# awkrail/svpc

Hardware: AMD Instinct MI355X
Metric: train steps/sec (vivt, batch=16, clip_seq=12) (higher is better)
Workload: dtype bf16x3; 1 GPU; MODEL_TYPE=vivt train step: N=16 videos/GPU x S=12 clips x Lv=100 frames x F=3072, Lt=22, D=768, H=12, L=6 (enc+step-enc+dec), V=951, A=384, E=10; dropout .1/.1/.4; fwd+bwd+allreduce+clip+BertAdam; mode=bf16x3, global_batch=16, parallelism=dp1, launch=hipGraph replay, gpus_requested=1

## Files before the change

include/svpc_hip.h:

```cpp
#ifndef SVPC_HIP_H
#define SVPC_HIP_H
#include <stddef.h>
#ifdef __cplusplus
extern "C" {
#endif

typedef struct ihipStream_t* svpc_stream_t;
typedef unsigned long long svpc_u64;

#define SVPC_ACT_NONE 0
#define SVPC_ACT_RELU 1
#define SVPC_ACT_GELU 2
#define SVPC_ACT_SIGMOID 3

const char* svpc_last_error(void);
int svpc_abi_version(void);

int svpc_ln_fwd(const float* x, const int* src_rows, const float* res, const float* gamma, const float* beta, float* y,
                float* mean, float* rstd, int R, int D, float eps, float p_pre, unsigned site_pre, float p_post,
                unsigned site_post, const svpc_u64* seed, const float* add1, int mod1, const float* add2, const int* idx2,
                svpc_stream_t stream);
int svpc_ln_fwd_t(const void* x, int x_dt, const int* src_rows, const void* res, const float* gamma, const float* beta, void* y,
                  int y_dt, float* mean, float* rstd, int R, int D, float eps, float p_pre, unsigned site_pre, float p_post,
                  unsigned site_post, const svpc_u64* seed, const float* add1, int mod1, const float* add2, const int* idx2,
// ... 64 lines not shown
int svpc_gemm_p8t(const void* A, int lda, const void* B, int ldb, void* C, int ldc, const void* G, int gact, const void* R, int M, int N, int K,
                  svpc_stream_t stream);
int svpc_gemm_l32_supported(int a_kc, int b_kc, int lda, int ldb, int M, int N, int K);
int svpc_gemm_l32_preferred(int a_kc, int b_kc, int lda, int ldb, int M, int N, int K);
int svpc_gemm_l32(const float* A, int lda, int a_kc, const float* B, int ldb, int b_kc, float* C, int ldc, float* Z, int M, int N, int K,
                  const float* bias, int act, float p_drop, unsigned site, const svpc_u64* seed, int accumulate, float* workspace,
                  size_t workspace_bytes, svpc_stream_t stream);
int svpc_gemm_l32_r(const float* A, int lda, int a_kc, const float* B, int ldb, int b_kc, float* C, int ldc, float* Z, const float* R, int M,
                    int N, int K, const float* bias, int act, float p_drop, unsigned site, const svpc_u64* seed, int accumulate,
                    float* workspace, size_t workspace_bytes, svpc_stream_t stream);
int svpc_gemm_l32_rg(const float* A, int lda, int a_kc, const float* B, int ldb, int b_kc, float* C, int ldc, const float* R, const float* G,
                     int gact, int M, int N, int K, int accumulate, float* workspace, size_t workspace_bytes, svpc_stream_t stream);
int svpc_gemm_l32_x3(const float* A, int lda, int a_kc, const float* B, int ldb, int b_kc, float* C, int ldc, float* Z, const float* R, int M,
                     int N, int K, const float* bias, int act, float p_drop, unsigned site, const svpc_u64* seed, int accumulate,
                     float* workspace, size_t workspace_bytes, svpc_stream_t stream);
typedef struct svpc_gemm_problem { const float* A; const float* B; float* C; int M, N, K, lda, ldb, ldc; } svpc_gemm_problem;
int svpc_gemm_group(const svpc_gemm_problem* problems, int n, int a_kc, int b_kc, int accumulate, svpc_stream_t stream);
int svpc_gemm_group_x3(const svpc_gemm_problem* problems, int n, int a_kc, int b_kc, int accumulate, svpc_stream_t stream);
typedef struct svpc_wgrad_problem {
    const float* dz; const float* x; float* dw; float* db;
    int n_out, n_in, rows, ld_dz, ld_x, ld_dw;
} svpc_wgrad_problem;
int svpc_gemm_group_wgrad_max(void);
int svpc_gemm_group_wgrad_bf16_p8_ok(const void* problems, int n);
int svpc_gemm_group_wgrad_bf16_p8(const void* problems, int n, float* workspace, size_t workspace_bytes, svpc_stream_t stream);
int svpc_gemm_group_wgrad_bf16(const svpc_wgrad_problem* problems, int n, svpc_stream_t stream);
int svpc_gemm_group_wgrad_bf16_ws(const svpc_wgrad_problem* problems, int n, float* workspace, size_t workspace_bytes,
                                  svpc_stream_t stream);
int svpc_gemm_group_wgrad(const svpc_wgrad_problem* problems, int n, svpc_stream_t stream);
int svpc_act_bwd(const float* dy, const float* aux, float* dz, size_t n, int act, float p, unsigned site, const svpc_u64* seed,
// ... 262 lines not shown
int svpc_scatter_add_rows_bf16(const float* rows, const int* idx, void* table, int ld_table, int R, int W, svpc_stream_t stream);
int svpc_pair_rows(float* a, const int* ia, float* b, const int* ib, float* out, float* out2, int R, int W, int mode, svpc_stream_t stream);
int svpc_add_cast_bf16(const void* a, const float* b, void* out, size_t n, svpc_stream_t stream);
int svpc_rows_expand(const float* src, const int* inv, float* out, int n_rows, int W, svpc_stream_t stream);
int svpc_add(const float* a, const float* b, float* c, size_t n, svpc_stream_t stream);
int svpc_sum_all(const float* x, size_t n, float* out, float scale, svpc_stream_t stream);
int svpc_fill_from(float* x, size_t n, const float* v, svpc_stream_t stream);
int svpc_dropout_mask(float* out, size_t n, float p, unsigned site, const svpc_u64* seed, svpc_stream_t stream);
int svpc_attn_dropout_mask(float* out, size_t n_rows, int max_k, float p, unsigned site, const svpc_u64* seed, svpc_stream_t stream);
int svpc_bump_seed(svpc_u64* seed, svpc_stream_t stream);

int svpc_opt_chunk(void);
int svpc_opt_meta_bytes(void);
int svpc_opt_step(const void* meta, const int* chunk_tid, const long long* chunk_start, const int* tensor_chunk_off, int n_tensors,
                  int n_chunks, float* partial, float* norms_sq, const float* hyper, svpc_stream_t stream);
int svpc_opt_zero_grad(const void* meta, const int* chunk_tid, const long long* chunk_start, int n_chunks, svpc_stream_t stream);

#ifdef __cplusplus
}
#endif
#endif
```

svpc_amd/csrc/gemm_l32.hip:

```cpp
#include "gemm_common.h"
#include <stdlib.h>

typedef __bf16 bf16x8 __attribute__((ext_vector_type(8)));
typedef const void __attribute__((address_space(1))) * l32_gptr;
typedef void __attribute__((address_space(3))) * l32_lptr;

constexpr int L32_BK = 32;
__device__ __attribute__((aligned(16))) const float l32_zeros[4] = {0.f, 0.f, 0.f, 0.f};

template <int N> __device__ __forceinline__ void l32_wait_vmcnt() { asm volatile("s_waitcnt vmcnt(%0)" ::"n"(N) : "memory"); }

template <int R, bool KC>
__device__ __forceinline__ const float* l32_src(const float* P, int ld, int m0, int rows, int k0, int j, int lane) {
    if (KC) {
        const int row = 8 * j + (lane >> 3), pos = lane & 7;
        const int c = pos ^ ((row >> 1) & 7);
        const int gr = min(m0 + row, rows - 1);
        return P + (size_t)gr * ld + k0 + 4 * c;
    } else {
        constexpr int CPR = R / 4;
        const int krow = j * (64 / CPR) + lane / CPR, c = lane % CPR;
        const int gm = min(m0 + 4 * c, rows - 4);
        return P + (size_t)(k0 + krow) * ld + gm;
    }
// ... 38 lines not shown
    } else {
        const float* p = reinterpret_cast<const float*>(img) + (16 * ks + 8 * (lane >> 5)) * R + row0 + (lane & 31);
#pragma unroll
        for (int j = 0; j < 8; ++j) f[j] = p[j * R];
    }
    l32_split8(f, hi, lo);
}
#define L32_MFMA3(ah, al, bh, bl, acc)                                           \
    do {                                                                         \
        acc = __builtin_amdgcn_mfma_f32_32x32x16_bf16(al, bh, acc, 0, 0, 0);     \
        acc = __builtin_amdgcn_mfma_f32_32x32x16_bf16(ah, bl, acc, 0, 0, 0);     \
        acc = __builtin_amdgcn_mfma_f32_32x32x16_bf16(ah, bh, acc, 0, 0, 0);     \
    } while (0)


template <int BM, int BN, bool A_KC, bool B_KC, int NS, bool X3 = false>
__global__ __launch_bounds__(256) void gemm_l32_kernel(const float* __restrict__ A, int lda, const float* __restrict__ B, int ldb,
                                                       float* __restrict__ C, int ldc, int M, int N, int K, Epi epi, int tiles_m,
                                                       int tiles_n, int splitk, int k_chunk, float* __restrict__ slabs, int remap) {
    extern __shared__ __attribute__((aligned(1024))) char l32_smem[];
    constexpr int A_BYTES = BM * L32_BK * 4, B_BYTES = BN * L32_BK * 4, STAGE = A_BYTES + B_BYTES;
    constexpr int A_PER_WAVE = BM / 32, B_PER_WAVE = BN / 32;
    constexpr int P = A_PER_WAVE + B_PER_WAVE;
    constexpr int TM = BM / 64, TN = BN / 64;
    const int wg = remap ? xcd_remap(blockIdx.x, tiles_m * tiles_n * splitk) : (int)blockIdx.x;
    const int ks_id = wg / (tiles_m * tiles_n);
    const int tile = wg - ks_id * (tiles_m * tiles_n);
    const int tm = tile / tiles_n, tn = tile - tm * tiles_n;
    const int m0 = tm * BM, n0 = tn * BN;
    const int k_begin = ks_id * k_chunk;
    const int k_end = min(K, k_begin + k_chunk);
    const int nk = (k_end - k_begin + L32_BK - 1) / L32_BK;
    const int k_tail = (k_end - k_begin) - (nk - 1) * L32_BK;

    const int lane = threadIdx.x & 63, wave = threadIdx.x >> 6;
    const int wr = wave >> 1, wc = wave & 1;

    const float* ga[A_PER_WAVE];
    const float* gb[B_PER_WAVE];
#pragma unroll
// ... 90 lines not shown
                    const int row = m0 + wr * (BM / 2) + i * 32 + (e & 3) + 8 * (e >> 2) + 4 * lhi;
                    vs[e] = acc[i][j][e]; oks[e] = row < M && col < N; rs[e] = min(row, M - 1); cs[e] = min(col, N - 1);
                }
                epilogue_store_n<16>(vs, rs, cs, oks, C, ldc, epi, seed, inv_keep);
                continue;
            }
            if (col >= N) continue;
#pragma unroll
            for (int e = 0; e < 16; ++e) {
                const int row = m0 + wr * (BM / 2) + i * 32 + (e & 3) + 8 * (e >> 2) + 4 * lhi;
                if (row >= M) continue;
                slabs[((size_t)ks_id * M + row) * N + col] = acc[i][j][e];
            }
        }
}

template <bool A_KC, bool B_KC, int NS = 2, bool X3 = false, bool PRE = false>
__device__ __forceinline__ void l32w_tile(char* l32_smem, const float* __restrict__ A, int lda, const float* __restrict__ B, int ldb,
                                          float* __restrict__ C, int ldc, int M, int N, int K, const Epi& epi, int tm, int tn,
                                          float* __restrict__ asum) {
    constexpr int T = 64, OP = T * L32_BK * 4, STAGE = 2 * OP, PIECES = OP / 1024;
    const int m0 = tm * T, n0 = tn * T;
    float cpre[PRE ? T * T / 256 : 1];
    if constexpr (PRE) {
#pragma unroll
        for (int u = 0; u < T * T / 256; ++u) {
            const int idx = threadIdx.x + 256 * u;
            const int row = m0 + (idx >> 6), col = n0 + (idx & 63);
            cpre[u] = (row < M && col < N) ? C[(size_t)row * ldc + col] : 0.f;
        }
// ... 298 lines not shown
        float v = part[0][e][l];
#pragma unroll
        for (int w = 1; w < NW; ++w) v += part[w][e][l];
        vs[i] = v;
        oks[i] = row < ts && col < ts && m0 + row < M && n0 + col < N;
        rs[i] = min(m0 + row, M - 1); cs[i] = min(n0 + col, N - 1);
    }
    epilogue_store_n<NE>(vs, rs, cs, oks, C, ldc, epi, seed, inv_keep);
}
template <bool B_KC, bool X3 = false>
__global__ __launch_bounds__(256) void gemm_skinny_kernel(const float* __restrict__ A, int lda, const float* __restrict__ B, int ldb,
                                                          float* __restrict__ C, int ldc, int M, int N, int K, Epi epi, int tiles_n, int ts) {
    __shared__ float part[4][16][64];
    const int tm = blockIdx.x / tiles_n, tn = blockIdx.x - tm * tiles_n;
    skinny_tile<B_KC, 4, X3>(part, A, lda, B, ldb, C, ldc, M, N, K, epi, tm, tn, ts);
}
template <int NW, bool X3 = false, bool B_KC = true>
__global__ __launch_bounds__(64 * NW) void gemm_group_skinny_kernel(GemmGroupArgs g) {
    __shared__ float part[NW][16][64];
    int pi = 0;
    while (pi + 1 < g.n && (int)blockIdx.x >= g.p[pi + 1].tile0) ++pi;
    const GemmProb& q = g.p[pi];
    const int tile = blockIdx.x - q.tile0;
    const int tm = tile / q.tiles_n, tn = tile - tm * q.tiles_n;
    Epi epi{nullptr, ACT_NONE, 0.f, 0u, nullptr, g.accumulate, nullptr};
    skinny_tile<B_KC, NW, X3>(part, q.A, q.lda, q.B, q.ldb, q.C, q.ldc, q.M, q.N, q.K, epi, tm, tn);
}

struct LstmStep {
    const float* h_prev[2]; const float* c_prev[2]; const float* w_hh[2]; const float* gx[2]; const int* rows[2]; const float* active;
// ... 171 lines not shown
        hipError_t e = hipFuncSetAttribute(reinterpret_cast<const void*>(&gemm_group_wgrad_kernel<2>), hipFuncAttributeMaxDynamicSharedMemorySize,
                                           LDS2);
        if (e == hipSuccess)
            e = hipFuncSetAttribute(reinterpret_cast<const void*>(&gemm_group_wgrad_kernel<1>), hipFuncAttributeMaxDynamicSharedMemorySize, LDS1);
        if (e != hipSuccess) { svpc_set_error("gemm_group_wgrad: cannot raise the dynamic LDS limit"); return (int)e; }
        attr_set = true;
    }
    static int ns_env = -1;
    if (ns_env < 0) { const char* e = getenv("SVPC_GROUP_WGRAD_NS"); ns_env = e ? atoi(e) : 1; }
    const bool one_stage = ns_env != 2;
    if (one_stage) hipLaunchKernelGGL(gemm_group_wgrad_kernel<1>, dim3(tiles), dim3(256), LDS1, stream, g);
    else hipLaunchKernelGGL(gemm_group_wgrad_kernel<2>, dim3(tiles), dim3(256), LDS2, stream, g);
    return svpc_check_launch("gemm_group_wgrad");
}

static int gemm_l32_x(const float* A, int lda, int a_kc, const float* B, int ldb, int b_kc, float* C, int ldc, float* Z, const float* R,
                      const float* G, int gact, int M, int N, int K, const float* bias, int act, float p_drop, unsigned site, const u64* seed,
                      int accumulate, float* workspace, size_t workspace_bytes, int x3, hipStream_t stream);
int svpc_gemm_l32_r(const float* A, int lda, int a_kc, const float* B, int ldb, int b_kc, float* C, int ldc, float* Z, const float* R, int M,
                    int N, int K, const float* bias, int act, float p_drop, unsigned site, const u64* seed, int accumulate,
                    float* workspace, size_t workspace_bytes, hipStream_t stream) {
    return gemm_l32_x(A, lda, a_kc, B, ldb, b_kc, C, ldc, Z, R, nullptr, ACT_NONE, M, N, K, bias, act, p_drop, site, seed, accumulate, workspace,
                      workspace_bytes, 0, stream);
}
int svpc_gemm_l32_rg(const float* A, int lda, int a_kc, const float* B, int ldb, int b_kc, float* C, int ldc, const float* R, const float* G,
                     int gact, int M, int N, int K, int accumulate, float* workspace, size_t workspace_bytes, hipStream_t stream) {
    return gemm_l32_x(A, lda, a_kc, B, ldb, b_kc, C, ldc, nullptr, R, G, gact, M, N, K, nullptr, ACT_NONE, 0.f, 0u, nullptr, accumulate,
                      workspace, workspace_bytes, 0, stream);
}
int svpc_gemm_l32_x3(const float* A, int lda, int a_kc, const float* B, int ldb, int b_kc, float* C, int ldc, float* Z, const float* R, int M,
                     int N, int K, const float* bias, int act, float p_drop, unsigned site, const u64* seed, int accumulate,
                     float* workspace, size_t workspace_bytes, hipStream_t stream) {
    return gemm_l32_x(A, lda, a_kc, B, ldb, b_kc, C, ldc, Z, R, nullptr, ACT_NONE, M, N, K, bias, act, p_drop, site, seed, accumulate, workspace,
                      workspace_bytes, 1, stream);
}
int svpc_gemm_l32(const float* A, int lda, int a_kc, const float* B, int ldb, int b_kc, float* C, int ldc, float* Z, int M, int N, int K,
                  const float* bias, int act, float p_drop, unsigned site, const u64* seed, int accumulate, float* workspace,
                  size_t workspace_bytes, hipStream_t stream) {
    return svpc_gemm_l32_r(A, lda, a_kc, B, ldb, b_kc, C, ldc, Z, nullptr, M, N, K, bias, act, p_drop, site, seed, accumulate, workspace,
                           workspace_bytes, stream);
}
}
static int gemm_l32_x(const float* A, int lda, int a_kc, const float* B, int ldb, int b_kc, float* C, int ldc, float* Z, const float* R,
                      const float* G, int gact, int M, int N, int K, const float* bias, int act, float p_drop, unsigned site, const u64* seed,
                      int accumulate, float* workspace, size_t workspace_bytes, int x3, hipStream_t stream) {
    if (M == 0 || N == 0) return 0;
    SVPC_REQUIRE(svpc_gemm_l32_supported(a_kc, b_kc, lda, ldb, M, N, K) && ((((uintptr_t)A) | ((uintptr_t)B)) & 15) == 0,
                 "gemm_l32: needs K % 32 == 0 (or both operands k-contiguous and K % 4 == 0) and 16-byte aligned fp32 rows");
    SVPC_REQUIRE(p_drop <= 0.f || seed != nullptr, "gemm: dropout needs a seed pointer");
    Epi epi{bias, act, p_drop, site, seed, accumulate, Z, R, G, gact};
    static int env_tile = -1, env_split = -1, remap = -1;
    if (env_tile < 0) { const char* e = getenv("SVPC_L32_TILE"); env_tile = e ? atoi(e) : 0; }
    if (env_split < 0) { const char* e = getenv("SVPC_L32_SPLITK"); env_split = e ? atoi(e) : 0; }
    if (remap < 0) { const char* e = getenv("SVPC_GEMM_REMAP"); remap = e ? atoi(e) : 1; }
    static int env_skinny = -1;
    if (env_skinny < 0) { const char* e = getenv("SVPC_L32_SKINNY"); env_skinny = e ? atoi(e) : 1; }
    static int skinny_m = -1;
    if (skinny_m < 0) { const char* e = getenv("SVPC_L32_SKINNY_M"); skinny_m = e ? atoi(e) : 256; }
    if (env_skinny && a_kc && M <= skinny_m && N >= 32 && (K & 15) == 0 && (lda & 3) == 0 && (!b_kc || (ldb & 3) == 0)) {
        static int env_ts = -1;
        if (env_ts < 0) { const char* e = getenv("SVPC_L32_SKINNY_TS"); env_ts = e ? atoi(e) : 24; }
        const int t24 = ceil_div(M, 24) * ceil_div(N, 24), t32 = ceil_div(M, 32) * ceil_div(N, 32);
        const int ts = (env_ts == 24 && t24 <= 256 && t32 < t24 && t32 > 64) ? 24 : 32;
        const int tn_ = ceil_div(N, ts);
        dim3 grids(ceil_div(M, ts) * tn_);
        if (x3) {
            if (b_kc) hipLaunchKernelGGL((gemm_skinny_kernel<true, true>), grids, dim3(256), 0, stream, A, lda, B, ldb, C, ldc, M, N, K, epi, tn_, ts);
            else hipLaunchKernelGGL((gemm_skinny_kernel<false, true>), grids, dim3(256), 0, stream, A, lda, B, ldb, C, ldc, M, N, K, epi, tn_, ts);
        } else if (b_kc) hipLaunchKernelGGL((gemm_skinny_kernel<true, false>), grids, dim3(256), 0, stream, A, lda, B, ldb, C, ldc, M, N, K, epi, tn_, ts);
        else hipLaunchKernelGGL((gemm_skinny_kernel<false, false>), grids, dim3(256), 0, stream, A, lda, B, ldb, C, ldc, M, N, K, epi, tn_, ts);
        return svpc_check_launch("gemm_skinny");
    }
    const int t128 = ceil_div(M, 128) * ceil_div(N, 128), t64 = ceil_div(M, 64) * ceil_div(N, 64);
    int mode = (M >= 96 && N >= 96 && t128 > 300) ? 128 : 65;
    static int env_w = -1;
    if (env_w < 0) { const char* e = getenv("SVPC_L32_WAVESPLIT"); env_w = e ? atoi(e) : 1; }
    if (env_w && t64 <= 256 && K >= 4 * L32_BK) mode = 66;
    if (env_tile == 128 || env_tile == 64 || env_tile == 65 || env_tile == 66) mode = env_tile;
    const bool k_tail = K % L32_BK != 0;
    if (k_tail && (mode == 66 || mode == 64)) mode = 65;
    if (mode == 66) {
        const int tm_ = ceil_div(M, 64), tn_ = ceil_div(N, 64);
        dim3 gridw(tm_ * tn_);
        int rcw;
        if (x3) {
            if (a_kc && b_kc) rcw = l32w_launch_one<true, true, true>(gridw, stream, A, lda, B, ldb, C, ldc, M, N, K, epi, tm_, tn_);
            else if (a_kc) rcw = l32w_launch_one<true, false, true>(gridw, stream, A, lda, B, ldb, C, ldc, M, N, K, epi, tm_, tn_);
            else if (b_kc) rcw = l32w_launch_one<false, true, true>(gridw, stream, A, lda, B, ldb, C, ldc, M, N, K, epi, tm_, tn_);
            else rcw = l32w_launch_one<false, false, true>(gridw, stream, A, lda, B, ldb, C, ldc, M, N, K, epi, tm_, tn_);
        } else if (a_kc && b_kc) rcw = l32w_launch_one<true, true>(gridw, stream, A, lda, B, ldb, C, ldc, M, N, K, epi, tm_, tn_);
        else if (a_kc) rcw = l32w_launch_one<true, false>(gridw, stream, A, lda, B, ldb, C, ldc, M, N, K, epi, tm_, tn_);
        else if (b_kc) rcw = l32w_launch_one<false, true>(gridw, stream, A, lda, B, ldb, C, ldc, M, N, K, epi, tm_, tn_);
        else rcw = l32w_launch_one<false, false>(gridw, stream, A, lda, B, ldb, C, ldc, M, N, K, epi, tm_, tn_);
        if (rcw) return rcw;
        return svpc_check_launch("gemm_l32w");
// ... 36 lines not shown
```

svpc_amd/csrc/optimizer.hip:

```cpp
#include "common.h"

struct TensorMeta { float* p; float* g; float* m; float* v; float* ema; long long n; float wd; int pad; __bf16* shadow; __bf16* shadow_lo; };

constexpr int OPT_CHUNK = 16384;

__global__ __launch_bounds__(256) void opt_sumsq_kernel(const TensorMeta* __restrict__ meta, const int* __restrict__ chunk_tid,
                                                        const long long* __restrict__ chunk_start, float* __restrict__ partial) {
    __shared__ float red[4];
    const int c = blockIdx.x;
    const TensorMeta t = meta[chunk_tid[c]];
    const long long s = chunk_start[c];
    const long long e = s + OPT_CHUNK < t.n ? s + OPT_CHUNK : t.n;
    float acc = 0.f;
    if ((e - s) == OPT_CHUNK && ((((unsigned long long)(t.g + s)) & 15ull) == 0)) {
        const float4* g4 = reinterpret_cast<const float4*>(t.g + s);
        float4 v[OPT_CHUNK / 4 / 256];
#pragma unroll
        for (int k = 0; k < OPT_CHUNK / 4 / 256; ++k) v[k] = g4[threadIdx.x + 256 * k];
#pragma unroll
        for (int k = 0; k < OPT_CHUNK / 4 / 256; ++k) acc += v[k].x * v[k].x + v[k].y * v[k].y + v[k].z * v[k].z + v[k].w * v[k].w;
    } else {
        for (long long i = s + threadIdx.x; i < e; i += 256) { const float g = t.g[i]; acc += g * g; }
    }
    acc = block_sum_256(acc, red);
    if (threadIdx.x == 0) partial[c] = acc;
}
__global__ __launch_bounds__(256) void opt_norms_kernel(const float* __restrict__ partial, const int* __restrict__ tensor_chunk_off,
                                                        int n_tensors, float* __restrict__ norms_sq) {
    __shared__ float red[4];
    float tot = 0.f;
    for (int t = threadIdx.x; t < n_tensors; t += 256) {
        float s = 0.f;
        for (int c = tensor_chunk_off[t]; c < tensor_chunk_off[t + 1]; ++c) s += partial[c];
        norms_sq[t] = s;
        tot += s;
    }
    tot = block_sum_256(tot, red);
    if (threadIdx.x == 0) norms_sq[n_tensors] = tot;
}
__global__ __launch_bounds__(256) void opt_adam_kernel(const TensorMeta* __restrict__ meta, const int* __restrict__ chunk_tid,
                                                       const long long* __restrict__ chunk_start, const float* __restrict__ norms_sq,
                                                       int n_tensors, const float* __restrict__ hyper) {
    const int c = blockIdx.x;
    const int tid = chunk_tid[c];
    const TensorMeta t = meta[tid];
    const float lr = hyper[0], ema_decay = hyper[1], max_g = hyper[2], max_t = hyper[3], b1 = hyper[4], b2 = hyper[5], eps = hyper[6];
    float coef = 1.0f;
    if (max_g > 0.f) coef = fminf(1.0f, max_g / (sqrtf(norms_sq[n_tensors]) + 1e-6f));
    if (max_t > 0.f) {
        const float tn = sqrtf(norms_sq[tid]) * coef;
// ... 77 lines not shown
}
__global__ __launch_bounds__(256) void opt_zero_kernel(const TensorMeta* __restrict__ meta, const int* __restrict__ chunk_tid,
                                                       const long long* __restrict__ chunk_start) {
    const int c = blockIdx.x;
    const TensorMeta t = meta[chunk_tid[c]];
    const long long s = chunk_start[c];
    const long long e = s + OPT_CHUNK < t.n ? s + OPT_CHUNK : t.n;
    for (long long i = s + threadIdx.x; i < e; i += 256) t.g[i] = 0.f;
}

extern "C" {

int svpc_opt_chunk(void) { return OPT_CHUNK; }
int svpc_opt_meta_bytes(void) { return (int)sizeof(TensorMeta); }

int svpc_opt_step(const void* meta, const int* chunk_tid, const long long* chunk_start, const int* tensor_chunk_off, int n_tensors,
                  int n_chunks, float* partial, float* norms_sq, const float* hyper, hipStream_t s) {
    if (n_chunks == 0) return 0;
    hipLaunchKernelGGL(opt_sumsq_kernel, dim3(n_chunks), dim3(256), 0, s, (const TensorMeta*)meta, chunk_tid, chunk_start, partial);
    int rc = svpc_check_launch("opt_sumsq");
    if (rc) return rc;
    hipLaunchKernelGGL(opt_norms_kernel, dim3(1), dim3(256), 0, s, partial, tensor_chunk_off, n_tensors, norms_sq);
    rc = svpc_check_launch("opt_norms");
    if (rc) return rc;
    hipLaunchKernelGGL(opt_adam_kernel, dim3(n_chunks), dim3(256), 0, s, (const TensorMeta*)meta, chunk_tid, chunk_start, norms_sq,
                       n_tensors, hyper);
    return svpc_check_launch("opt_adam");
}
int svpc_opt_zero_grad(const void* meta, const int* chunk_tid, const long long* chunk_start, int n_chunks, hipStream_t s) {
    if (n_chunks == 0) return 0;
    hipLaunchKernelGGL(opt_zero_kernel, dim3(n_chunks), dim3(256), 0, s, (const TensorMeta*)meta, chunk_tid, chunk_start);
    return svpc_check_launch("opt_zero");
}

}
```

svpc_amd/model.py:

```python
from __future__ import annotations

import math

import numpy as np
import torch
import torch.nn as nn

from . import ops
from .ops_common import ACT_GELU, ACT_NONE, ACT_RELU, ACT_SIGMOID, BulkUpload, FIdx, Idx

PAD_ROW = 0


def _sinusoid(max_len, d):
    pe = torch.zeros(max_len, d)
    pos = torch.arange(0, max_len).float().unsqueeze(1)
    div = torch.exp(torch.arange(0, d, 2).float() * -(math.log(10000.0) / d))
    pe[:, 0::2] = torch.sin(pos * div)
    pe[:, 1::2] = torch.cos(pos * div)
    return pe


def _i32(v, device):
    return torch.tensor(v, dtype=torch.int32, device=device)
# ... 983 lines not shown
        return torch.cat(out, 0).contiguous()

    @staticmethod
    def _padded_bank(ents, plan):
        D = ents.shape[1]
        per_vid = []
        for b in range(plan.N):
            e = ents[plan.h_ent_off[b]:plan.h_ent_off[b] + plan.h_ent_len[b]]
            if plan.h_ent_len[b] < plan.e_max:
                e = torch.cat([e, e.new_zeros(plan.e_max - plan.h_ent_len[b], D)], 0)
            per_vid.append(e.unsqueeze(0).expand(plan.h_step_len[b], -1, -1))
        return torch.cat(per_vid, 0).contiguous()

    def _bilstm(self, x, plan):
        rnn = self.recipe_encoder
        gx, whh = [], []
        pairs = [(getattr(rnn, "bias_ih_l0" + sfx), getattr(rnn, "bias_hh_l0" + sfx)) for sfx in ("", "_reverse")]
        direct = [ops.direct_grads(bi, bh) for bi, bh in pairs]
        if all(d is not None for d in direct) and x.is_cuda:
            with torch.no_grad():
                sums = torch._foreach_add([p[0] for p in pairs], [p[1] for p in pairs])
        else:
            sums = [bi + bh for bi, bh in pairs]
        for z, sfx in enumerate(("", "_reverse")):
            w_ih, w_hh = getattr(rnn, "weight_ih_l0" + sfx), getattr(rnn, "weight_hh_l0" + sfx)
            gx.append(ops.linear(x, w_ih, sums[z], bgrad=direct[z]))
            whh.append(w_hh)
        return ops.bilstm_sequences(gx[0], gx[1], whh[0], whh[1], plan.lstm_fwd_rows, plan.lstm_bwd_rows, plan.lstm_active,
                                    plan.lstm_pick[""], plan.lstm_pick["_reverse"], summed=True)

    def reconstruct(self, prediction_scores, text_mask, ga_ingr_vectors):
        S, Lt, C = prediction_scores.shape
        dev = prediction_scores.device
        cx = self._cx(dev)
        E = ga_ingr_vectors.shape[0]
        plan = BatchPlan([S], [E], S, 1, self.config.max_v_len, Lt, self.config.max_v_len + Lt, self._n_mem(), dev)
        noise = None if self.gumbel_noise is None else self.gumbel_noise[0].reshape(S * Lt, C)
        bow = ops.gumbel_bow(prediction_scores.reshape(S * Lt, C).contiguous(), Idx([C] * (S * Lt)),
                             self.text_embeddings.word_embeddings.weight, self.config.temperature,
                             noise=noise, rng=cx.rng, site=cx.rng.site())
        pooled = ops.span_mean(bow, plan.text_starts, plan.text_lens, weights=text_mask.reshape(-1).float())
        return self.recipe_reasoner.run(self._bilstm(pooled, plan), ga_ingr_vectors.contiguous(), plan.sim, cx)
# ... 4 lines not shown
```

svpc_amd/ops.py:

```python
from __future__ import annotations

import ctypes
import math
import numbers
import os
import struct

import torch
from torch.autograd import Function as _TorchFunction

from . import _lib
from .ops_common import ACT_GELU, ACT_NONE, ACT_RELU, ACT_SIGMOID, FIdx, Idx, SeqInfo, as_idx

_WS = {}
_WS_BYTES = 256 << 20


_DEV_IDX = [None]


def _stream():
    i = _DEV_IDX[0]
    if i is None or not _FAST_STREAM:
        return torch.cuda.current_stream().cuda_stream
# ... 946 lines not shown
    if tok_in is not None and (trans_w or not can_g):
        tok_in = None
    y = _Linear.apply(x, w, b, act, trans_w, drop, wgrad, bgrad, w16, tok_out, tok_in)
    if split:
        y._svpc_lo = y.shape[1]
    if abl and "o" in abl:
        if split:
            _lo_view(y).zero_()
        else:
            y = y.to(torch.bfloat16).float()
    if tok_out is not None:
        y._svpc_act_tok = tok_out
    return y


class _LayerNorm(Function):
    @staticmethod
    def forward(ctx, x, gamma, beta, residual, add2, eps, src_rows, pad_row, pre_drop, post_drop, add1, add1_mod, add2_idx,
                out_bf16=False, sink=False, out_split=False):
        _need_gpu(x)
        ctx.sink = bool(sink)
        ctx.direct = (_direct(gamma), _direct(beta), _direct(x) if src_rows is not None else None,
                      _direct(add2) if add2 is not None else None)
        x_lo = lo_off(x)
        r_lo = lo_off(residual) if residual is not None else None
        split = out_split or x_lo is not None or r_lo is not None
        if x_lo is None:
            x = _c(x)
        D = x.shape[1]
        R = src_rows.numel() if src_rows is not None else x.shape[0]
# ... 2146 lines not shown
```

svpc_amd/optim.py:

```python
from __future__ import annotations

import ctypes
import re

import torch

from . import _lib

NO_DECAY = ("bias", "LayerNorm.bias", "LayerNorm.weight")


def warmup_linear(progress, warmup):
    if progress < warmup:
        return progress / warmup
    return max((progress - 1.0) / (warmup - 1.0), 0.0)


WEIGHTS_EPOCH = [0]


class _Meta(ctypes.Structure):
    _fields_ = [("p", ctypes.c_void_p), ("g", ctypes.c_void_p), ("m", ctypes.c_void_p), ("v", ctypes.c_void_p),
                ("ema", ctypes.c_void_p), ("n", ctypes.c_longlong), ("wd", ctypes.c_float), ("pad", ctypes.c_int),
                ("shadow", ctypes.c_void_p), ("shadow_lo", ctypes.c_void_p)]
# ... 272 lines not shown
    def set_hyper(self):
        h = self._hyper_host
        h[0] = self.scheduled_lr()
        h[1] = min(self.ema_decay, (1.0 + self.step_count) / (10.0 + self.step_count)) if self.ema_decay >= 0 else -1.0
        h[2] = self.grad_clip if self.grad_clip and self.grad_clip > 0 else -1.0
        h[3] = self.max_grad_norm if self.max_grad_norm and self.max_grad_norm > 0 else -1.0
        h[4], h[5], h[6] = self.b1, self.b2, self.eps
        self.hyper.copy_(h, non_blocking=True)

    def launch(self):
        from . import clip_graphs, ops
        clip_graphs.check_consumed()
        WEIGHTS_EPOCH[0] += 1
        ops.join_side()
        stream = torch.cuda.current_stream().cuda_stream
        _lib.call("opt_step", self.meta.data_ptr(), self.chunk_tid.data_ptr(), self.chunk_start.data_ptr(),
                  self.tensor_chunk_off.data_ptr(), self.n_tensors, self.n_chunks, self.partial.data_ptr(),
                  self.norms_sq.data_ptr(), self.hyper.data_ptr(), stream)

    def step(self):
        self.ensure_built()
        self.set_hyper()
        self.launch()
        self.step_count += 1

    def ema_assign(self):
        assert self.ema is not None and self.arena is not None
        WEIGHTS_EPOCH[0] += 1
        self._backup = self.weights.flat.clone()
        with torch.no_grad():
            self.weights.flat.copy_(self.ema)
        self.weights.refresh()

# ... 205 lines not shown
```

Measured before the change: 90.38 steps/s (one step = 16 clip-sequences per GPU; whole-job aggregate).

## Pair BiLSTM input projections into one GEMM launch and stage optimizer norm reduction in LDS

The forward and reverse BiLSTM input projections share the same input and shape. They now run as a single paired GEMM launch with twice the grid, and their data-gradient GEMMs in backward are paired the same way. This is meant to cut launch count and fill more of the GPU for these small GEMMs. Separately, the optimizer's per-tensor norm reduction now stages chunk partials through shared memory in coalesced batches instead of each thread reading its own strided run. Both paths carry new env toggles, and the tile-planning logic is moved into a shared helper.

```diff
diff --git a/include/svpc_hip.h b/include/svpc_hip.h
--- a/include/svpc_hip.h
+++ b/include/svpc_hip.h
@@ -102,6 +102,9 @@
 int svpc_gemm_l32_x3(const float* A, int lda, int a_kc, const float* B, int ldb, int b_kc, float* C, int ldc, float* Z, const float* R, int M,
                      int N, int K, const float* bias, int act, float p_drop, unsigned site, const svpc_u64* seed, int accumulate,
                      float* workspace, size_t workspace_bytes, svpc_stream_t stream);
+int svpc_gemm_l32_pair_ok(int a_kc, int b_kc, int lda, int ldb, int M, int N, int K);
+int svpc_gemm_l32_pair(const float* A0, const float* B0, float* C0, const float* bias0, const float* A1, const float* B1, float* C1,
+                       const float* bias1, int lda, int a_kc, int ldb, int b_kc, int ldc, int M, int N, int K, int x3, svpc_stream_t stream);
 typedef struct svpc_gemm_problem { const float* A; const float* B; float* C; int M, N, K, lda, ldb, ldc; } svpc_gemm_problem;
 int svpc_gemm_group(const svpc_gemm_problem* problems, int n, int a_kc, int b_kc, int accumulate, svpc_stream_t stream);
 int svpc_gemm_group_x3(const svpc_gemm_problem* problems, int n, int a_kc, int b_kc, int accumulate, svpc_stream_t stream);
@@ -394,6 +397,8 @@
 int svpc_opt_meta_bytes(void);
 int svpc_opt_step(const void* meta, const int* chunk_tid, const long long* chunk_start, const int* tensor_chunk_off, int n_tensors,
                   int n_chunks, float* partial, float* norms_sq, const float* hyper, svpc_stream_t stream);
+int svpc_opt_step_ex(const void* meta, const int* chunk_tid, const long long* chunk_start, const int* tensor_chunk_off, int n_tensors,
+                     int n_chunks, float* partial, float* norms_sq, const float* hyper, int staged_norms, svpc_stream_t stream);
 int svpc_opt_zero_grad(const void* meta, const int* chunk_tid, const long long* chunk_start, int n_chunks, svpc_stream_t stream);
 
 #ifdef __cplusplus
diff --git a/svpc_amd/csrc/gemm_l32.hip b/svpc_amd/csrc/gemm_l32.hip
--- a/svpc_amd/csrc/gemm_l32.hip
+++ b/svpc_amd/csrc/gemm_l32.hip
@@ -76,16 +76,14 @@
     } while (0)
 
 
-template <int BM, int BN, bool A_KC, bool B_KC, int NS, bool X3 = false>
-__global__ __launch_bounds__(256) void gemm_l32_kernel(const float* __restrict__ A, int lda, const float* __restrict__ B, int ldb,
-                                                       float* __restrict__ C, int ldc, int M, int N, int K, Epi epi, int tiles_m,
-                                                       int tiles_n, int splitk, int k_chunk, float* __restrict__ slabs, int remap) {
-    extern __shared__ __attribute__((aligned(1024))) char l32_smem[];
+template <int BM, int BN, bool A_KC, bool B_KC, int NS, bool X3>
+__device__ __forceinline__ void l32_tile_run(char* l32_smem, const float* __restrict__ A, int lda, const float* __restrict__ B, int ldb,
+                                             float* __restrict__ C, int ldc, int M, int N, int K, const Epi& epi, int tiles_m, int tiles_n,
+                                             int splitk, int k_chunk, float* __restrict__ slabs, int wg) {
     constexpr int A_BYTES = BM * L32_BK * 4, B_BYTES = BN * L32_BK * 4, STAGE = A_BYTES + B_BYTES;
     constexpr int A_PER_WAVE = BM / 32, B_PER_WAVE = BN / 32;
     constexpr int P = A_PER_WAVE + B_PER_WAVE;
     constexpr int TM = BM / 64, TN = BN / 64;
-    const int wg = remap ? xcd_remap(blockIdx.x, tiles_m * tiles_n * splitk) : (int)blockIdx.x;
     const int ks_id = wg / (tiles_m * tiles_n);
     const int tile = wg - ks_id * (tiles_m * tiles_n);
     const int tm = tile / tiles_n, tn = tile - tm * tiles_n;
@@ -206,6 +204,27 @@
             }
         }
 }
+template <int BM, int BN, bool A_KC, bool B_KC, int NS, bool X3 = false>
+__global__ __launch_bounds__(256) void gemm_l32_kernel(const float* __restrict__ A, int lda, const float* __restrict__ B, int ldb,
+                                                       float* __restrict__ C, int ldc, int M, int N, int K, Epi epi, int tiles_m,
+                                                       int tiles_n, int splitk, int k_chunk, float* __restrict__ slabs, int remap) {
+    extern __shared__ __attribute__((aligned(1024))) char l32_smem[];
+    const int wg = remap ? xcd_remap(blockIdx.x, tiles_m * tiles_n * splitk) : (int)blockIdx.x;
+    l32_tile_run<BM, BN, A_KC, B_KC, NS, X3>(l32_smem, A, lda, B, ldb, C, ldc, M, N, K, epi, tiles_m, tiles_n, splitk, k_chunk, slabs, wg);
+}
+struct L32Pair { const float* A0; const float* B0; float* C0; const float* bias0; const float* A1; const float* B1; float* C1; const float* bias1; };
+template <int BM, int BN, bool A_KC, bool B_KC, int NS, bool X3>
+__global__ __launch_bounds__(256) void gemm_l32_pair_kernel(L32Pair q, int lda, int ldb, int ldc, int M, int N, int K, int tiles_m, int tiles_n,
+                                                            int remap) {
+    extern __shared__ __attribute__((aligned(1024))) char l32_smem[];
+    const int tiles = tiles_m * tiles_n;
+    int wg = remap ? xcd_remap(blockIdx.x, 2 * tiles) : (int)blockIdx.x;
+    const bool z = wg >= tiles;
+    if (z) wg -= tiles;
+    const Epi epi{z ? q.bias1 : q.bias0, ACT_NONE, 0.f, 0u, nullptr, 0, nullptr};
+    l32_tile_run<BM, BN, A_KC, B_KC, NS, X3>(l32_smem, z ? q.A1 : q.A0, lda, z ? q.B1 : q.B0, ldb, z ? q.C1 : q.C0, ldc, M, N, K, epi, tiles_m,
+                                             tiles_n, 1, K, nullptr, wg);
+}
 
 template <bool A_KC, bool B_KC, int NS = 2, bool X3 = false, bool PRE = false>
 __device__ __forceinline__ void l32w_tile(char* l32_smem, const float* __restrict__ A, int lda, const float* __restrict__ B, int ldb,
@@ -534,6 +553,16 @@
     __shared__ float part[4][16][64];
     const int tm = blockIdx.x / tiles_n, tn = blockIdx.x - tm * tiles_n;
     skinny_tile<B_KC, 4, X3>(part, A, lda, B, ldb, C, ldc, M, N, K, epi, tm, tn, ts);
+}
+template <bool B_KC, bool X3>
+__global__ __launch_bounds__(256) void gemm_skinny_pair_kernel(L32Pair q, int lda, int ldb, int ldc, int M, int N, int K, int tiles_n, int tiles,
+                                                               int ts) {
+    __shared__ float part[4][16][64];
+    const bool z = (int)blockIdx.x >= tiles;
+    const int tile = (int)blockIdx.x - (z ? tiles : 0);
+    const int tm = tile / tiles_n, tn = tile - tm * tiles_n;
+    const Epi epi{z ? q.bias1 : q.bias0, ACT_NONE, 0.f, 0u, nullptr, 0, nullptr};
+    skinny_tile<B_KC, 4, X3>(part, z ? q.A1 : q.A0, lda, z ? q.B1 : q.B0, ldb, z ? q.C1 : q.C0, ldc, M, N, K, epi, tm, tn, ts);
 }
 template <int NW, bool X3 = false, bool B_KC = true>
 __global__ __launch_bounds__(64 * NW) void gemm_group_skinny_kernel(GemmGroupArgs g) {
@@ -735,6 +764,36 @@
     return svpc_check_launch("gemm_group_wgrad");
 }
 
+struct L32Plan { int skinny, ts, mode, remap, env_split; };
+static L32Plan l32_plan(int a_kc, int b_kc, int lda, int ldb, int M, int N, int K) {
+    static int env_tile = -1, env_split = -1, remap = -1;
+    if (env_tile < 0) { const char* e = getenv("SVPC_L32_TILE"); env_tile = e ? atoi(e) : 0; }
+    if (env_split < 0) { const char* e = getenv("SVPC_L32_SPLITK"); env_split = e ? atoi(e) : 0; }
+    if (remap < 0) { const char* e = getenv("SVPC_GEMM_REMAP"); remap = e ? atoi(e) : 1; }
+    static int env_skinny = -1;
+    if (env_skinny < 0) { const char* e = getenv("SVPC_L32_SKINNY"); env_skinny = e ? atoi(e) : 1; }
+    static int skinny_m = -1;
+    if (skinny_m < 0) { const char* e = getenv("SVPC_L32_SKINNY_M"); skinny_m = e ? atoi(e) : 256; }
+    L32Plan pl{0, 32, 65, remap, env_split};
+    if (env_skinny && a_kc && M <= skinny_m && N >= 32 && (K & 15) == 0 && (lda & 3) == 0 && (!b_kc || (ldb & 3) == 0)) {
+        static int env_ts = -1;
+        if (env_ts < 0) { const char* e = getenv("SVPC_L32_SKINNY_TS"); env_ts = e ? atoi(e) : 24; }
+        const int t24 = ceil_div(M, 24) * ceil_div(N, 24), t32 = ceil_div(M, 32) * ceil_div(N, 32);
+        pl.skinny = 1;
+        pl.ts = (env_ts == 24 && t24 <= 256 && t32 < t24 && t32 > 64) ? 24 : 32;
+        return pl;
+    }
+    const int t128 = ceil_div(M, 128) * ceil_div(N, 128), t64 = ceil_div(M, 64) * ceil_div(N, 64);
+    int mode = (M >= 96 && N >= 96 && t128 > 300) ? 128 : 65;
+    static int env_w = -1;
+    if (env_w < 0) { const char* e = getenv("SVPC_L32_WAVESPLIT"); env_w = e ? atoi(e) : 1; }
+    if (env_w && t64 <= 256 && K >= 4 * L32_BK) mode = 66;
+    if (env_tile == 128 || env_tile == 64 || env_tile == 65 || env_tile == 66) mode = env_tile;
+    if (K % L32_BK != 0 && (mode == 66 || mode == 64)) mode = 65;
+    pl.mode = mode;
+    return pl;
+}
+
 static int gemm_l32_x(const float* A, int lda, int a_kc, const float* B, int ldb, int b_kc, float* C, int ldc, float* Z, const float* R,
                       const float* G, int gact, int M, int N, int K, const float* bias, int act, float p_drop, unsigned site, const u64* seed,
                       int accumulate, float* workspace, size_t workspace_bytes, int x3, hipStream_t stream);
@@ -761,6 +820,52 @@
     return svpc_gemm_l32_r(A, lda, a_kc, B, ldb, b_kc, C, ldc, Z, nullptr, M, N, K, bias, act, p_drop, site, seed, accumulate, workspace,
                            workspace_bytes, stream);
 }
+int svpc_gemm_l32_pair_ok(int a_kc, int b_kc, int lda, int ldb, int M, int N, int K) {
+    if (!svpc_gemm_l32_supported(a_kc, b_kc, lda, ldb, M, N, K)) return 0;
+    const L32Plan pl = l32_plan(a_kc, b_kc, lda, ldb, M, N, K);
+    if (pl.skinny) return 1;
+    if (pl.mode != 65 || !(a_kc && b_kc) || pl.env_split > 0) return 0;
+    const int tiles = ceil_div(M, 64) * ceil_div(N, 64);
+    if (tiles <= 128 && K >= 2048 && K % L32_BK == 0) return 0;
+    return 1;
+}
+int svpc_gemm_l32_pair(const float* A0, const float* B0, float* C0, const float* bias0, const float* A1, const float* B1, float* C1,
+                       const float* bias1, int lda, int a_kc, int ldb, int b_kc, int ldc, int M, int N, int K, int x3, hipStream_t stream) {
+    if (M == 0 || N == 0) return 0;
+    SVPC_REQUIRE(svpc_gemm_l32_pair_ok(a_kc, b_kc, lda, ldb, M, N, K) &&
+                     ((((uintptr_t)A0) | ((uintptr_t)B0) | ((uintptr_t)A1) | ((uintptr_t)B1)) & 15) == 0,
+                 "gemm_l32_pair: a shape the single launch runs in its skinny or unsplit 64x64 tiled form, 16-byte aligned fp32 rows");
+    const L32Plan pl = l32_plan(a_kc, b_kc, lda, ldb, M, N, K);
+    const L32Pair q{A0, B0, C0, bias0, A1, B1, C1, bias1};
+    if (pl.skinny) {
+        const int ts = pl.ts, tn_ = ceil_div(N, ts), tiles = ceil_div(M, ts) * tn_;
+        dim3 grid(2 * tiles);
+        if (x3) {
+            if (b_kc) hipLaunchKernelGGL((gemm_skinny_pair_kernel<true, true>), grid, dim3(256), 0, stream, q, lda, ldb, ldc, M, N, K, tn_, tiles, ts);
+            else hipLaunchKernelGGL((gemm_skinny_pair_kernel<false, true>), grid, dim3(256), 0, stream, q, lda, ldb, ldc, M, N, K, tn_, tiles, ts);
+        } else if (b_kc) hipLaunchKernelGGL((gemm_skinny_pair_kernel<true, false>), grid, dim3(256), 0, stream, q, lda, ldb, ldc, M, N, K, tn_, tiles, ts);
+        else hipLaunchKernelGGL((gemm_skinny_pair_kernel<false, false>), grid, dim3(256), 0, stream, q, lda, ldb, ldc, M, N, K, tn_, tiles, ts);
+        return svpc_check_launch("gemm_skinny_pair");
+    }
+    const int tiles_m = ceil_div(M, 64), tiles_n = ceil_div(N, 64);
+    constexpr int LDS = 4 * (64 + 64) * L32_BK * 4;
+    static bool attr_set = false;
+    if (!attr_set) {
+        hipError_t e = hipFuncSetAttribute(reinterpret_cast<const void*>(&gemm_l32_pair_kernel<64, 64, true, true, 4, true>),
+                                           hipFuncAttributeMaxDynamicSharedMemorySize, LDS);
+        if (e == hipSuccess)
+            e = hipFuncSetAttribute(reinterpret_cast<const void*>(&gemm_l32_pair_kernel<64, 64, true, true, 4, false>),
+                                    hipFuncAttributeMaxDynamicSharedMemorySize, LDS);
+        if (e != hipSuccess) { svpc_set_error("gemm_l32_pair: cannot raise the dynamic LDS limit"); return (int)e; }
+        attr_set = true;
+    }
+    dim3 grid(2 * tiles_m * tiles_n);
+    if (x3) hipLaunchKernelGGL((gemm_l32_pair_kernel<64, 64, true, true, 4, true>), grid, dim3(256), LDS, stream, q, lda, ldb, ldc, M, N, K,
+                               tiles_m, tiles_n, pl.remap);
+    else hipLaunchKernelGGL((gemm_l32_pair_kernel<64, 64, true, true, 4, false>), grid, dim3(256), LDS, stream, q, lda, ldb, ldc, M, N, K,
+                            tiles_m, tiles_n, pl.remap);
+    return svpc_check_launch("gemm_l32_pair");
+}
 }
 static int gemm_l32_x(const float* A, int lda, int a_kc, const float* B, int ldb, int b_kc, float* C, int ldc, float* Z, const float* R,
                       const float* G, int gact, int M, int N, int K, const float* bias, int act, float p_drop, unsigned site, const u64* seed,
@@ -770,19 +875,10 @@
                  "gemm_l32: needs K % 32 == 0 (or both operands k-contiguous and K % 4 == 0) and 16-byte aligned fp32 rows");
     SVPC_REQUIRE(p_drop <= 0.f || seed != nullptr, "gemm: dropout needs a seed pointer");
     Epi epi{bias, act, p_drop, site, seed, accumulate, Z, R, G, gact};
-    static int env_tile = -1, env_split = -1, remap = -1;
-    if (env_tile < 0) { const char* e = getenv("SVPC_L32_TILE"); env_tile = e ? atoi(e) : 0; }
-    if (env_split < 0) { const char* e = getenv("SVPC_L32_SPLITK"); env_split = e ? atoi(e) : 0; }
-    if (remap < 0) { const char* e = getenv("SVPC_GEMM_REMAP"); remap = e ? atoi(e) : 1; }
-    static int env_skinny = -1;
-    if (env_skinny < 0) { const char* e = getenv("SVPC_L32_SKINNY"); env_skinny = e ? atoi(e) : 1; }
-    static int skinny_m = -1;
-    if (skinny_m < 0) { const char* e = getenv("SVPC_L32_SKINNY_M"); skinny_m = e ? atoi(e) : 256; }
-    if (env_skinny && a_kc && M <= skinny_m && N >= 32 && (K & 15) == 0 && (lda & 3) == 0 && (!b_kc || (ldb & 3) == 0)) {
-        static int env_ts = -1;
-        if (env_ts < 0) { const char* e = getenv("SVPC_L32_SKINNY_TS"); env_ts = e ? atoi(e) : 24; }
-        const int t24 = ceil_div(M, 24) * ceil_div(N, 24), t32 = ceil_div(M, 32) * ceil_div(N, 32);
-        const int ts = (env_ts == 24 && t24 <= 256 && t32 < t24 && t32 > 64) ? 24 : 32;
+    const L32Plan pl = l32_plan(a_kc, b_kc, lda, ldb, M, N, K);
+    const int remap = pl.remap, env_split = pl.env_split;
+    if (pl.skinny) {
+        const int ts = pl.ts;
         const int tn_ = ceil_div(N, ts);
         dim3 grids(ceil_div(M, ts) * tn_);
         if (x3) {
@@ -792,14 +888,8 @@
         else hipLaunchKernelGGL((gemm_skinny_kernel<false, false>), grids, dim3(256), 0, stream, A, lda, B, ldb, C, ldc, M, N, K, epi, tn_, ts);
         return svpc_check_launch("gemm_skinny");
     }
-    const int t128 = ceil_div(M, 128) * ceil_div(N, 128), t64 = ceil_div(M, 64) * ceil_div(N, 64);
-    int mode = (M >= 96 && N >= 96 && t128 > 300) ? 128 : 65;
-    static int env_w = -1;
-    if (env_w < 0) { const char* e = getenv("SVPC_L32_WAVESPLIT"); env_w = e ? atoi(e) : 1; }
-    if (env_w && t64 <= 256 && K >= 4 * L32_BK) mode = 66;
-    if (env_tile == 128 || env_tile == 64 || env_tile == 65 || env_tile == 66) mode = env_tile;
+    int mode = pl.mode;
     const bool k_tail = K % L32_BK != 0;
-    if (k_tail && (mode == 66 || mode == 64)) mode = 65;
     if (mode == 66) {
         const int tm_ = ceil_div(M, 64), tn_ = ceil_div(N, 64);
         dim3 gridw(tm_ * tn_);
diff --git a/svpc_amd/csrc/optimizer.hip b/svpc_amd/csrc/optimizer.hip
--- a/svpc_amd/csrc/optimizer.hip
+++ b/svpc_amd/csrc/optimizer.hip
@@ -34,6 +34,45 @@
         for (int c = tensor_chunk_off[t]; c < tensor_chunk_off[t + 1]; ++c) s += partial[c];
         norms_sq[t] = s;
         tot += s;
+    }
+    tot = block_sum_256(tot, red);
+    if (threadIdx.x == 0) norms_sq[n_tensors] = tot;
+}
+constexpr int OPT_STAGE = 8192;
+__global__ __launch_bounds__(256) void opt_norms_staged_kernel(const float* __restrict__ partial, const int* __restrict__ tensor_chunk_off,
+                                                               int n_tensors, float* __restrict__ norms_sq) {
+    __shared__ float red[4];
+    __shared__ float stage[OPT_STAGE];
+    float tot = 0.f;
+    for (int base = 0; base < n_tensors; base += 256) {
+        const int t = base + threadIdx.x;
+        const bool live = t < n_tensors;
+        const int c0 = live ? tensor_chunk_off[t] : 0, c1 = live ? tensor_chunk_off[t + 1] : 0;
+        const int lo = tensor_chunk_off[base], hi = tensor_chunk_off[min(base + 256, n_tensors)];
+        float s = 0.f;
+        for (int w = lo; w < hi; w += OPT_STAGE) {
+            const int n = min(OPT_STAGE, hi - w);
+            __syncthreads();
+            for (int i0 = threadIdx.x; i0 < n; i0 += 256 * 8) {
+                float v[8];
+#pragma unroll
+                for (int k = 0; k < 8; ++k) v[k] = partial[w + min(i0 + 256 * k, n - 1)];
+#pragma unroll
+                for (int k = 0; k < 8; ++k) if (i0 + 256 * k < n) stage[i0 + 256 * k] = v[k];
+            }
+            __syncthreads();
+            const int b = min(c1, w + n) - w;
+            int c = max(c0, w) - w;
+            for (; c + 8 <= b; c += 8) {
+                float v[8];
+#pragma unroll
+                for (int k = 0; k < 8; ++k) v[k] = stage[c + k];
+#pragma unroll
+                for (int k = 0; k < 8; ++k) s += v[k];
+            }
+            for (; c < b; ++c) s += stage[c];
+        }
+        if (live) { norms_sq[t] = s; tot += s; }
     }
     tot = block_sum_256(tot, red);
     if (threadIdx.x == 0) norms_sq[n_tensors] = tot;
@@ -141,19 +180,24 @@
 int svpc_opt_chunk(void) { return OPT_CHUNK; }
 int svpc_opt_meta_bytes(void) { return (int)sizeof(TensorMeta); }
 
-int svpc_opt_step(const void* meta, const int* chunk_tid, const long long* chunk_start, const int* tensor_chunk_off, int n_tensors,
-                  int n_chunks, float* partial, float* norms_sq, const float* hyper, hipStream_t s) {
+int svpc_opt_step_ex(const void* meta, const int* chunk_tid, const long long* chunk_start, const int* tensor_chunk_off, int n_tensors,
+                     int n_chunks, float* partial, float* norms_sq, const float* hyper, int staged_norms, hipStream_t s) {
     if (n_chunks == 0) return 0;
     hipLaunchKernelGGL(opt_sumsq_kernel, dim3(n_chunks), dim3(256), 0, s, (const TensorMeta*)meta, chunk_tid, chunk_start, partial);
     int rc = svpc_check_launch("opt_sumsq");
     if (rc) return rc;
-    hipLaunchKernelGGL(opt_norms_kernel, dim3(1), dim3(256), 0, s, partial, tensor_chunk_off, n_tensors, norms_sq);
+    if (staged_norms) hipLaunchKernelGGL(opt_norms_staged_kernel, dim3(1), dim3(256), 0, s, partial, tensor_chunk_off, n_tensors, norms_sq);
+    else hipLaunchKernelGGL(opt_norms_kernel, dim3(1), dim3(256), 0, s, partial, tensor_chunk_off, n_tensors, norms_sq);
     rc = svpc_check_launch("opt_norms");
     if (rc) return rc;
     hipLaunchKernelGGL(opt_adam_kernel, dim3(n_chunks), dim3(256), 0, s, (const TensorMeta*)meta, chunk_tid, chunk_start, norms_sq,
                        n_tensors, hyper);
     return svpc_check_launch("opt_adam");
 }
+int svpc_opt_step(const void* meta, const int* chunk_tid, const long long* chunk_start, const int* tensor_chunk_off, int n_tensors,
+                  int n_chunks, float* partial, float* norms_sq, const float* hyper, hipStream_t s) {
+    return svpc_opt_step_ex(meta, chunk_tid, chunk_start, tensor_chunk_off, n_tensors, n_chunks, partial, norms_sq, hyper, 1, s);
+}
 int svpc_opt_zero_grad(const void* meta, const int* chunk_tid, const long long* chunk_start, int n_chunks, hipStream_t s) {
     if (n_chunks == 0) return 0;
     hipLaunchKernelGGL(opt_zero_kernel, dim3(n_chunks), dim3(256), 0, s, (const TensorMeta*)meta, chunk_tid, chunk_start);
diff --git a/svpc_amd/model.py b/svpc_amd/model.py
--- a/svpc_amd/model.py
+++ b/svpc_amd/model.py
@@ -1021,7 +1021,6 @@
 
     def _bilstm(self, x, plan):
         rnn = self.recipe_encoder
-        gx, whh = [], []
         pairs = [(getattr(rnn, "bias_ih_l0" + sfx), getattr(rnn, "bias_hh_l0" + sfx)) for sfx in ("", "_reverse")]
         direct = [ops.direct_grads(bi, bh) for bi, bh in pairs]
         if all(d is not None for d in direct) and x.is_cuda:
@@ -1029,10 +1028,13 @@
                 sums = torch._foreach_add([p[0] for p in pairs], [p[1] for p in pairs])
         else:
             sums = [bi + bh for bi, bh in pairs]
-        for z, sfx in enumerate(("", "_reverse")):
-            w_ih, w_hh = getattr(rnn, "weight_ih_l0" + sfx), getattr(rnn, "weight_hh_l0" + sfx)
-            gx.append(ops.linear(x, w_ih, sums[z], bgrad=direct[z]))
-            whh.append(w_hh)
+        wih = [getattr(rnn, "weight_ih_l0" + sfx) for sfx in ("", "_reverse")]
+        whh = [getattr(rnn, "weight_hh_l0" + sfx) for sfx in ("", "_reverse")]
+        pair = getattr(ops, "linear_pair", None)
+        if pair is not None:
+            gx = pair(x, wih, sums, bgrads=direct)
+        else:
+            gx = [ops.linear(x, wih[z], sums[z], bgrad=direct[z]) for z in range(2)]
         return ops.bilstm_sequences(gx[0], gx[1], whh[0], whh[1], plan.lstm_fwd_rows, plan.lstm_bwd_rows, plan.lstm_active,
                                     plan.lstm_pick[""], plan.lstm_pick["_reverse"], summed=True)
 
diff --git a/svpc_amd/ops.py b/svpc_amd/ops.py
--- a/svpc_amd/ops.py
+++ b/svpc_amd/ops.py
@@ -984,6 +984,92 @@
     return y
 
 
+PAIR_LSTM_PROJ = os.environ.get("SVPC_PAIR_LSTM_PROJ", "1") != "0"
+OPT_NORMS_STAGED = os.environ.get("SVPC_OPT_NORMS_STAGED", "1") != "0"
+
+
+class _LinearCtx:
+
+    def __init__(self, needs_input_grad):
+        self.needs_input_grad = needs_input_grad
+        self.saved_tensors = ()
+
+    def save_for_backward(self, *tensors):
+        self.saved_tensors = tensors
+
+
+def _pair_route_ok(A, lda, B, ldb, b_kc, M, N, K, x3):
+    lib = _lib.load()
+    if not (_fast() and not BWD_EXACT and (A.data_ptr() | B.data_ptr()) % 16 == 0):
+        return False
+    if x3:
+        single = lib.svpc_gemm_l32_supported(1, b_kc, lda, ldb, M, N, K) == 1
+    else:
+        single = USE_L32 and lib.svpc_gemm_l32_preferred(1, b_kc, lda, ldb, M, N, K) == 1
+    return single and lib.svpc_gemm_l32_pair_ok(1, b_kc, lda, ldb, M, N, K) == 1
+
+
+class _LinearPair(Function):
+    @staticmethod
+    def forward(ctx, x, w0, w1, b0, b1, wgrad0, wgrad1, bgrad0, bgrad1):
+        _need_gpu(x)
+        x = _rows2d(x)
+        ws, bs = [_c(w0), _c(w1)], [b0, b1]
+        M, K = x.shape
+        N = ws[0].shape[0]
+        ys = [torch.empty(M, N, dtype=torch.float32, device=x.device) for _ in range(2)]
+        if ws[0].stride(0) == ws[1].stride(0) and _pair_route_ok(x, x.stride(0), ws[0], ws[0].stride(0), 1, M, N, K, is_x3()) and \
+                ws[1].data_ptr() % 16 == 0 and all(b is None or b.is_contiguous() for b in bs):
+            _lib.call("gemm_l32_pair", _p(x), _p(ws[0]), _p(ys[0]), _p(bs[0]), _p(x), _p(ws[1]), _p(ys[1]), _p(bs[1]), x.stride(0), 1,
+                      ws[0].stride(0), 1, N, M, N, K, 1 if is_x3() else 0, _stream())
+        else:
+            for z in range(2):
+                _gemm(x, x.stride(0), 1, ws[z], ws[z].stride(0), 1, ys[z], M, N, K, bias=bs[z], x3=is_x3())
+        ctx.save_for_backward(x, ws[0], ws[1])
+        ctx.has_b = [b is not None for b in bs]
+        ctx.direct = [(wgrad0, bgrad0), (wgrad1, bgrad1)]
+        return ys[0], ys[1]
+
+    @staticmethod
+    def backward(ctx, dy0, dy1):
+        x, w0, w1 = ctx.saved_tensors
+        ws, dys = [w0, w1], [_c(dy0), _c(dy1)]
+        M, K = x.shape
+        N = w0.shape[0]
+        need = ctx.needs_input_grad
+        paired = need[0] and not (_RES_SINK and x.data_ptr() in _RES_SINK) and w0.stride(0) == w1.stride(0) and \
+            _pair_route_ok(dys[0], N, w0, w0.stride(0), 0, M, K, N, False) and (dys[1].data_ptr() | w1.data_ptr()) % 16 == 0
+        dxs = [None, None]
+        if paired:
+            dxs = [torch.empty(M, K, dtype=torch.float32, device=x.device) for _ in range(2)]
+            _lib.call("gemm_l32_pair", _p(dys[0]), _p(w0), _p(dxs[0]), None, _p(dys[1]), _p(w1), _p(dxs[1]), None, N, 1, w0.stride(0), 0, K,
+                      M, K, N, 0, _stream())
+        dws, dbs = [None, None], [None, None]
+        for z in (1, 0):
+            c = _LinearCtx((need[0] and not paired, need[1 + z], need[3 + z]))
+            c.saved_tensors = (x, ws[z], None)
+            c.cfg = (ACT_NONE, False, 0.0, 0, None, ctx.has_b[z])
+            c.direct = ctx.direct[z]
+            c.tok_out = c.tok_in = None
+            r = _Linear.backward(c, dys[z])
+            if not paired:
+                dxs[z] = r[0]
+            dws[z], dbs[z] = r[1], r[2]
+        dx = dxs[1].add_(dxs[0]) if need[0] else None
+        return dx, dws[0], dws[1], dbs[0], dbs[1], None, None, None, None
+
+
+def linear_pair(x, ws, bs, bgrads=(None, None)):
+    ok = (PAIR_LSTM_PROJ and x.is_cuda and x.dtype == torch.float32 and x.dim() == 2 and lo_off(x) is None and _fast() and not BWD_EXACT
+          and getattr(x, "_svpc_act_tok", None) is None and ABLATE is None and GEMM_TIMER is None
+          and ws[0].shape == ws[1].shape and all(w.dtype == torch.float32 and w.dim() == 2 for w in ws)
+          and all(b is None or b.dtype == torch.float32 for b in bs))
+    if not ok:
+        return tuple(linear(x, ws[z], bs[z], bgrad=bgrads[z]) for z in range(2))
+    bg = [bgrads[z] if (bgrads[z] is not None or bs[z] is None) else _direct(bs[z]) for z in range(2)]
+    return _LinearPair.apply(x, ws[0], ws[1], bs[0], bs[1], _direct(ws[0]), _direct(ws[1]), bg[0], bg[1])
+
+
 class _LayerNorm(Function):
     @staticmethod
     def forward(ctx, x, gamma, beta, residual, add2, eps, src_rows, pad_row, pre_drop, post_drop, add1, add1_mod, add2_idx,
diff --git a/svpc_amd/optim.py b/svpc_amd/optim.py
--- a/svpc_amd/optim.py
+++ b/svpc_amd/optim.py
@@ -310,9 +310,9 @@
         WEIGHTS_EPOCH[0] += 1
         ops.join_side()
         stream = torch.cuda.current_stream().cuda_stream
-        _lib.call("opt_step", self.meta.data_ptr(), self.chunk_tid.data_ptr(), self.chunk_start.data_ptr(),
+        _lib.call("opt_step_ex", self.meta.data_ptr(), self.chunk_tid.data_ptr(), self.chunk_start.data_ptr(),
                   self.tensor_chunk_off.data_ptr(), self.n_tensors, self.n_chunks, self.partial.data_ptr(),
-                  self.norms_sq.data_ptr(), self.hyper.data_ptr(), stream)
+                  self.norms_sq.data_ptr(), self.hyper.data_ptr(), 1 if ops.OPT_NORMS_STAGED else 0, stream)
 
     def step(self):
         self.ensure_built()
```

After: 90.29 steps/s (one step = 16 clip-sequences per GPU; whole-job aggregate). About the same (-0.1%).
